# malcolmgreaves/deequ

Measured on AMD Instinct MI355X. Metric: rows/sec (whole node) for fused 16-col profile scan; % of HBM peak BW, higher is better.
Workload: dtype f64+int64+utf8; 1 GPU; C5 fused 16-col profile scan (8 f64 + 4 i64 + 4 utf8, 10% nulls) + state merge + incremental StateLoader append; rows_per_gpu=1000000000, chunk_rows=125000000, analyzers=93, parallelism=row-shard x1

## Files before the change

deequ_amd/csrc/dq_device.h:

```cpp
#pragma once

#include <cstdint>

namespace dq {

constexpr int kBlock = 256;
constexpr int kWaves = kBlock / 64;
constexpr int kRowsPerLane = 8;
constexpr int kRowsPerIter = kBlock * kRowsPerLane;
constexpr int kMaxWG = 4096;
constexpr int kTargetWGs = 8192;
constexpr int kMaxCols = 64;
constexpr int kMaxColTasks = 256;
constexpr int kMaxSchemaCols = 1 << 16;
constexpr int kMaxWhere = 8;
constexpr int kHllCopies = 8;
constexpr int kPredAccCopies = 16;
constexpr int kMaxRoots = 32;
constexpr int kMaxCounters = 32;
constexpr int kMaxInstr = 96;
constexpr int kPredStack = 16;
constexpr int kMaxRegexWords = 32768;

enum ColKind : int32_t {
// ... 77 lines not shown
};

struct alignas(16) ColPartial {
  double n, mean, m2;
  double sum;
  int64_t isum;
  int64_t count;
  int64_t nan_count;
  double fmin, fmax;
  int64_t pinf_count;
  int64_t ninf_count;
  int64_t isum_hi;
};
static_assert(sizeof(ColPartial) == 96, "ColPartial layout");

struct alignas(16) CorrPartial {
  double n, xa, ya, ck, xm, ym, pad0, pad1;
};
static_assert(sizeof(CorrPartial) == 64, "CorrPartial layout");

struct alignas(16) PredPartial {
  int64_t t[kMaxCounters];
  int64_t nn[kMaxCounters];
};

enum PredOp : int32_t {
  PO_ATOM_CMP = 1,
  PO_ATOM_ISNULL = 2,
  PO_ATOM_NOTNULL = 3,
  PO_CONST = 4,
// ... 58 lines not shown
```

deequ_amd/csrc/dq_kernels.hip:

```cpp
#include <hip/hip_runtime.h>

#include <cstdint>
#include <type_traits>

#include "dq_device.h"
#include "dq_hash.h"
#include "dq_decimal.h"
#include "dq_lane.h"
#include "dq_shift.h"

namespace dq {

#define DQ_DEC_TABLE static __constant__ const
#include "dq_dec_tables.inc"
#undef DQ_DEC_TABLE
__device__ __forceinline__ DecTab dec_dev_tab() { return DecTab{kDecP10Lo, kDecP10Hi, kDecRcpHi, kDecRcpLo}; }

typedef uint32_t u32x4 __attribute__((ext_vector_type(4)));

__device__ __forceinline__ uint32_t ld32(const uint8_t* base, int64_t a) {
  return *reinterpret_cast<const uint32_t*>(base + a);
}
__device__ __forceinline__ uint32_t read4(const uint8_t* base, int64_t pos) {
  int64_t a = pos & ~int64_t(3);
// ... 75 lines not shown
__device__ __forceinline__ uint32_t hll_hi_from_fmix(uint64_t b) {
  const uint32_t bl = (uint32_t)b, bh = (uint32_t)(b >> 32);
  return __umulhi(bl, (uint32_t)XP3) + bl * (uint32_t)(XP3 >> 32) + bh * (uint32_t)XP3;
}
__device__ __forceinline__ HllKey hll_key_from_fmix(uint64_t b) {
  const uint32_t hi = hll_hi_from_fmix(b);
  return {(hi >> 21) & 0x7FCu, ffbh_raw(hi << 9)};
}

constexpr int32_t kFloorMin = 13;
__device__ __forceinline__ uint32_t hll_floor_thr(const uint32_t* __restrict__ hll_floor, int32_t slot) {
  if (!hll_floor || slot < 0) return 0u;
  const int32_t qfloor = (int32_t)hll_floor[slot] - 1;
  return qfloor >= kFloorMin ? 1u << (31 - min(qfloor, 22)) : 0u;
}
__device__ __forceinline__ HllKey hll_key_long(uint64_t v) { return hll_key_from_fmix(xxh64_long_head(v)); }
__device__ __forceinline__ HllKey hll_key_int(uint32_t v) { return hll_key_from_fmix(xxh64_int_head(v)); }


struct ColStats {
  double n, mean, m2, sum;
  int64_t isum, count, nan_count;
  double fmin, fmax;
  int64_t pinf, ninf;
  int64_t isum_hi;
};

__device__ __forceinline__ void stats_init(ColStats& s) {
  s.n = 0.0; s.mean = 0.0; s.m2 = 0.0; s.sum = 0.0;
  s.isum = 0; s.count = 0; s.nan_count = 0;
// ... 169 lines not shown
    asm volatile(
        "s_and_saveexec_b64 %[save], %[ma]\n\t"
        "v_add_f64 %[d], %[x], -%[sh]\n\t"
        "v_add_f64 %[sd], %[sd], %[d]\n\t"
        "v_fma_f64 %[sdd], %[d], %[d], %[sdd]\n\t"
        "s_and_b64 exec, %[save], %[mb]\n\t"
        "v_min_f64 %[lo], %[lo], %[x]\n\t"
        "v_max_f64 %[hi], %[hi], %[x]\n\t"
        "s_mov_b64 exec, %[save]"
        : [sd] "+v"(a.sd), [sdd] "+v"(a.sdd), [lo] "+v"(lo), [hi] "+v"(hi), [d] "=&v"(d), [save] "=&s"(save)
        : [x] "v"(x), [sh] "s"(shift), [ma] "s"(ma), [mb] "s"(mb)
        : "scc");
  }
}

template <int KIND, bool STATS, bool HLL, bool FLOOR = false>
__device__ __forceinline__ void numeric_block(const double (&x)[8], const uint64_t (&bits)[8], const uint64_t (&m)[8],
                                              double shift, ColStats& s, LaneMoments& a, int32_t* regs, int32_t& qmin,
                                              uint32_t thr = 0) {
  uint32_t rmin = ~0u;
#pragma unroll
  for (int j = 0; j < 8; ++j) {
    if (STATS) masked_moments<!ck_float(KIND), false>(a, s.fmin, s.fmax, x[j], bits[j], shift, m[j], m[j]);
    if (HLL) {
      if constexpr (FLOOR) {
        const uint64_t b = ck_bytes(KIND) <= 4 ? xxh64_int_head((uint32_t)bits[j]) : xxh64_long_head(bits[j]);
        rmin = min(rmin, hll_hi_from_fmix(b) << 9);
      } else {
        const HllKey key = ck_bytes(KIND) <= 4 ? hll_key_int((uint32_t)bits[j]) : hll_key_long(bits[j]);
        qmin = min(qmin, key.q);
        if (lane_bit(m[j])) atomicMax(reinterpret_cast<int32_t*>(reinterpret_cast<char*>(regs) + key.addr), key.q);
      }
    }
  }
  if (HLL) {
    const bool redo = FLOOR ? rmin < thr : qmin < 0;
    if (__builtin_amdgcn_ballot_w64(redo) != 0) {
#pragma unroll 1
      for (int j = 0; j < 8; ++j) {
        if (lane_bit(m[j])) hll_update(regs, ck_bytes(KIND) <= 4 ? xxh64_int((uint32_t)bits[j]) : xxh64_long(bits[j]));
      }
      qmin = 0;
    }
  }
}

template <int KIND, bool STATS, bool HLL>
__device__ __forceinline__ void float_block_checked(__amdgpu_buffer_rsrc_t vr, const uint32_t* validity,
                                                    const uint32_t* mask, int64_t base, int32_t rem, int32_t vo,
                                                    double shift, ColStats& s, LaneMoments& a, int32_t* regs,
                                                    int64_t& cnt_w, int64_t& nan_v, int64_t& pinf_v, int64_t& ninf_v) {
  constexpr bool kF32 = KIND == CK_F32;
// ... 34 lines not shown
      if (lane_bit(mj)) {
        if (key.q >= 0) atomicMax(reinterpret_cast<int32_t*>(reinterpret_cast<char*>(regs) + key.addr), key.q);
        else hll_update(regs, kF32 ? xxh64_int((uint32_t)b) : xxh64_long(b));
      }
    }
  }
}

template <int K> struct KindT { using T = double; };
template <> struct KindT<CK_I64> { using T = int64_t; };
template <> struct KindT<CK_I32> { using T = int32_t; };
template <> struct KindT<CK_F32> { using T = float; };
template <> struct KindT<CK_I16> { using T = int16_t; };
template <> struct KindT<CK_I8> { using T = int8_t; };

template <int KIND, bool STATS, bool HLL>
__device__ void numeric_range(const void* values, const uint32_t* validity, const uint32_t* mask,
                              int64_t row0, int64_t row1, ColStats& s, int32_t* regs, uint32_t thr = 0) {
  using T = typename KindT<KIND>::T;
  constexpr bool kLazy = ck_float(KIND) && STATS;
  const int lane = threadIdx.x & 63;
  const int wave = __builtin_amdgcn_readfirstlane(threadIdx.x >> 6);
  const T* v = reinterpret_cast<const T*>(values);
  const __amdgpu_buffer_rsrc_t vr = __builtin_amdgcn_make_buffer_rsrc(
      const_cast<T*>(v + row0), (short)0, (int)((row1 - row0) * (int64_t)sizeof(T)), 0x00020000);
  int64_t nan_v = 0, pinf_v = 0, ninf_v = 0;
  int64_t cnt_w = 0;
  LaneMoments a{0.0, 0.0, 0};
  const double shift =
      STATS ? range_shift(validity, mask, row0, row1, lane, [=](int64_t r) { return range_value<KIND>(vr, r - row0); }) : 0.0;
  int32_t qmin = 0;
  const int32_t nr = (int32_t)(row1 - row0);
  auto block_loop = [&](auto floor_form) __attribute__((always_inline)) {
    constexpr bool FLOOR = decltype(floor_form)::value;
    for (int32_t rb = 0; rb < nr; rb += kRowsPerIter) {
      const int64_t base = row0 + rb + wave * 512;
      const int32_t rem = nr - rb - wave * 512;
      const bool full = rb + kRowsPerIter <= nr;
      uint64_t bits[8], m[8];
      double x[8];
      const int32_t vo = (rb + wave * 512 + lane) * (int32_t)sizeof(T);
#pragma unroll
      for (int j = 0; j < 8; ++j) {
        if constexpr (sizeof(T) == 8) {
          const auto w2 = __builtin_amdgcn_raw_buffer_load_b64(vr, vo + j * 512, 0, 2 );
          bits[j] = ((uint64_t)w2[1] << 32) | w2[0];
          if (KIND == CK_F64) x[j] = __builtin_bit_cast(double, bits[j]);
          else x[j] = __builtin_fma((double)(int32_t)w2[1], 4294967296.0, (double)w2[0]);
        } else if constexpr (KIND == CK_F32) {
// ... 9 lines not shown
          x[j] = (double)w;
        }
      }
      block_masks(validity, mask, base, rem, full, m);
      uint64_t nf_any = 0;
      if constexpr (ck_float(KIND) && !kLazy) {
#pragma unroll
        for (int j = 0; j < 8; ++j) nf_any |= __builtin_amdgcn_ballot_w64(!__builtin_isfinite(x[j])) & m[j];
      }
      if (ck_float(KIND) && !kLazy && nf_any != 0) {
        float_block_checked<KIND, STATS, HLL>(vr, validity, mask, base, rem, vo, shift, s, a, regs, cnt_w, nan_v, pinf_v,
                                              ninf_v);
      } else {
#pragma unroll
        for (int j = 0; j < 8; ++j) cnt_w += __builtin_popcountll(m[j]);
        numeric_block<KIND, STATS, HLL, FLOOR>(x, bits, m, shift, s, a, regs, qmin, thr);
      }
    }
  };
  if (HLL && thr != 0) block_loop(std::true_type{});
  else block_loop(std::false_type{});
  if constexpr (kLazy) {
    __shared__ int32_t redo;
    if (threadIdx.x == 0) redo = 0;
    __syncthreads();
    const bool bad = !__builtin_isfinite(a.sd) || !__builtin_isfinite(a.sdd);
    if (__builtin_amdgcn_ballot_w64(bad) != 0 && lane == 0) redo = 1;
    __syncthreads();
    if (redo) {
      if (HLL) {
        for (int i = threadIdx.x; i < 512; i += kBlock) regs[i] = -1;
      }
      stats_init(s);
      a = LaneMoments{0.0, 0.0, 0};
      cnt_w = 0;
      __syncthreads();
// ... 600 lines not shown
  }
  s.count += c;
}

template <int KIND, bool STATS, bool HLL>
__device__ void run_numeric(const ColTask& t, const ScanCols& cols, const ScanBitmaps& bm, int64_t row0, int64_t row1,
                            ColStats& s, int32_t* regs) {
  const uint32_t* mask = t.where >= 0 ? reinterpret_cast<const uint32_t*>(bm.where_bits[t.where]) : nullptr;
  numeric_range<KIND, STATS, HLL>(cols.values[t.col], cols.validity[t.col], mask, row0, row1, s, regs);
}

template <int V, bool LONG>
__device__ __forceinline__ void run_variant(const ColTask& t, const ScanCols& cols, const uint32_t* mask, int64_t row0,
                                            int64_t row1, int64_t n_rows, ColStats& s, int32_t* regs,
                                            const uint64_t* p5, uint32_t* dq, uint32_t* rare, uint32_t* cls,
                                            uint32_t thr) {
  const void* v = cols.values[t.col];
  const uint32_t* val = cols.validity[t.col];
  if constexpr (V == CV_VALIDITY) validity_range(val, mask, row0, row1, s);
  else if constexpr (V == CV_F64_S) numeric_range<CK_F64, true, false>(v, val, mask, row0, row1, s, regs);
  else if constexpr (V == CV_F64_SH) numeric_range<CK_F64, true, true>(v, val, mask, row0, row1, s, regs, thr);
  else if constexpr (V == CV_F64_H) numeric_range<CK_F64, false, true>(v, val, mask, row0, row1, s, regs, thr);
  else if constexpr (V == CV_I64_S) numeric_range<CK_I64, true, false>(v, val, mask, row0, row1, s, regs);
  else if constexpr (V == CV_I64_SH) numeric_range<CK_I64, true, true>(v, val, mask, row0, row1, s, regs, thr);
  else if constexpr (V == CV_I64_H) numeric_range<CK_I64, false, true>(v, val, mask, row0, row1, s, regs, thr);
  else if constexpr (V == CV_I32_S) numeric_range<CK_I32, true, false>(v, val, mask, row0, row1, s, regs);
  else if constexpr (V == CV_I32_SH) numeric_range<CK_I32, true, true>(v, val, mask, row0, row1, s, regs, thr);
  else if constexpr (V == CV_I32_H) numeric_range<CK_I32, false, true>(v, val, mask, row0, row1, s, regs, thr);
  else if constexpr (V == CV_F32_S) numeric_range<CK_F32, true, false>(v, val, mask, row0, row1, s, regs);
  else if constexpr (V == CV_F32_SH) numeric_range<CK_F32, true, true>(v, val, mask, row0, row1, s, regs, thr);
  else if constexpr (V == CV_F32_H) numeric_range<CK_F32, false, true>(v, val, mask, row0, row1, s, regs, thr);
  else if constexpr (V == CV_I16_S) numeric_range<CK_I16, true, false>(v, val, mask, row0, row1, s, regs);
  else if constexpr (V == CV_I16_SH) numeric_range<CK_I16, true, true>(v, val, mask, row0, row1, s, regs, thr);
  else if constexpr (V == CV_I16_H) numeric_range<CK_I16, false, true>(v, val, mask, row0, row1, s, regs, thr);
  else if constexpr (V == CV_I8_S) numeric_range<CK_I8, true, false>(v, val, mask, row0, row1, s, regs);
  else if constexpr (V == CV_I8_SH) numeric_range<CK_I8, true, true>(v, val, mask, row0, row1, s, regs, thr);
  else if constexpr (V == CV_I8_H) numeric_range<CK_I8, false, true>(v, val, mask, row0, row1, s, regs, thr);
  else if constexpr (V == CV_F64_D) float_dtype_range(reinterpret_cast<const double*>(v), val, mask, row0, row1, s);
  else if constexpr (V == CV_F32_D) float_dtype_range(reinterpret_cast<const float*>(v), val, mask, row0, row1, s);
  else if constexpr (V == CV_BOOL) bool_range(reinterpret_cast<const uint32_t*>(v), val, mask, row0, row1, s, regs);
  else if constexpr (V == CV_D128_S) decimal_range<true, false, false>(v, val, mask, row0, row1, s, regs, t.arg);
  else if constexpr (V == CV_D128_SH) decimal_range<true, true, false>(v, val, mask, row0, row1, s, regs, t.arg);
  else if constexpr (V == CV_D128_H) decimal_range<false, true, false>(v, val, mask, row0, row1, s, regs, t.arg);
  else if constexpr (V == CV_D128_D) decimal_range<false, false, true>(v, val, mask, row0, row1, s, regs, t.arg);
  else if constexpr (V == CV_UTF8_H || V == CV_UTF8_D || V == CV_UTF8_HD)
    utf8_range<int32_t, V != CV_UTF8_D, V != CV_UTF8_H, LONG>(
        reinterpret_cast<const uint8_t*>(v), reinterpret_cast<const int32_t*>(cols.offsets[t.col]), val, mask, row0,
        row1, n_rows, s, regs, p5, dq, rare, cls);
  else
    utf8_range<int64_t, V != CV_LUTF8_D, V != CV_LUTF8_H, LONG>(
        reinterpret_cast<const uint8_t*>(v), reinterpret_cast<const int64_t*>(cols.offsets[t.col]), val, mask, row0,
// ... 7 lines not shown
#define DQ_NUM_WAVES 6
#endif
template <int V, bool LONG>
constexpr int kMinWaves = V == CV_UTF8_H && !LONG && DQ_STR_CLS ? 5
                          : V == CV_UTF8_H && DQ_STR_WAVES > 0 ? DQ_STR_WAVES
                          : (V == CV_F64_SH || V == CV_I64_SH) && DQ_NUM_WAVES > 0 ? DQ_NUM_WAVES
                          : V == CV_LUTF8_H && LONG ? 5
                                                    : 1;

template <int V, bool LONG = false>
__global__ __launch_bounds__(kBlock) __attribute__((amdgpu_waves_per_eu(kMinWaves<V, LONG>))) void dq_column_scan(const ColTask* __restrict__ tasks, int32_t ntasks,
                                                         int32_t part_base, ScanCols cols, ScanBitmaps bm,
                                                         int64_t n_rows, int64_t rows_per_range,
                                                         ColPartial* __restrict__ partials,
                                                         uint32_t* __restrict__ hll_acc,
                                                         const uint32_t* __restrict__ hll_floor) {
  constexpr bool kHll = !(V == CV_VALIDITY || V == CV_F64_S || V == CV_I64_S || V == CV_I32_S || V == CV_F64_D ||
                         V == CV_UTF8_D || V == CV_LUTF8_D || V == CV_F32_S || V == CV_I16_S || V == CV_I8_S ||
                         V == CV_F32_D || V == CV_BOOL || V == CV_D128_S || V == CV_D128_D);
  constexpr bool kBool = V == CV_BOOL;
  constexpr bool kStr = V == CV_UTF8_H || V == CV_LUTF8_H || V == CV_UTF8_HD || V == CV_LUTF8_HD;
  __shared__ int32_t regs[kHll ? 512 : 2];
  __shared__ uint64_t p5[kStr ? 256 : 1];
  constexpr uint32_t kDCap = DQ_STR_CLS && (V == CV_UTF8_H || V == CV_LUTF8_H) && !LONG ? kDefCapCls : kDefCap;
  __shared__ uint32_t dfq[kStr ? kWaves * kDefFields * kDCap : 1];
  __shared__ uint32_t rare[kStr ? kWaves : 1];
  constexpr bool kCls = DQ_STR_CLS && (V == CV_UTF8_H || V == CV_LUTF8_H) && !LONG;
  __shared__ __attribute__((aligned(16))) uint32_t clsbuf[kCls ? kWaves * kClsWords : 4];
  __shared__ ColStats red[kWaves];
  const int32_t ti = blockIdx.x % ntasks;
  const int32_t range = blockIdx.x / ntasks;
  const ColTask t = tasks[ti];
  const int64_t row0 = (int64_t)range * rows_per_range;
  int64_t row1 = row0 + rows_per_range;
  if (row1 > n_rows) row1 = n_rows;
  if constexpr (kBool) {
    if (threadIdx.x < 2) regs[threadIdx.x] = 0;
    __syncthreads();
  }
  if constexpr (kHll) {
    for (int i = threadIdx.x; i < 512; i += kBlock) regs[i] = -1;
    if constexpr (kStr) {
      p5[threadIdx.x] = (uint64_t)threadIdx.x * XP5;
      if (threadIdx.x < kWaves) rare[threadIdx.x] = 0;
    }
    __syncthreads();
  }
  ColStats s;
  stats_init(s);
  const uint32_t* mask = t.where >= 0 ? reinterpret_cast<const uint32_t*>(bm.where_bits[t.where]) : nullptr;
  const int32_t wv = kStr ? __builtin_amdgcn_readfirstlane(threadIdx.x >> 6) : 0;
  run_variant<V, LONG>(t, cols, mask, row0, row1, n_rows, s, regs, p5, dfq + wv * kDefFields * kDCap, rare + wv,
                       clsbuf + (kCls ? wv * kClsWords : 0), kHll ? hll_floor_thr(hll_floor, t.hll_slot) : 0u);
  block_reduce_store(s, partials + (size_t)(part_base + ti) * kMaxWG + range, red);
  if constexpr (kStr) {
    if (threadIdx.x == 0 && bm.rare_rows) {
      uint32_t r = 0;
      for (int w = 0; w < kWaves; ++w) r += rare[w];
      if (r) atomicAdd(reinterpret_cast<unsigned long long*>(bm.rare_rows + part_base + ti), (unsigned long long)r);
    }
  }
  if constexpr (kBool) {
    if (threadIdx.x == 0 && t.hll_slot >= 0) {
      uint32_t* dst = hll_acc + ((size_t)t.hll_slot * kHllCopies + (blockIdx.x % kHllCopies)) * 512;
      for (int b = 0; b < 2; ++b) {
        if (!regs[b]) continue;
        const uint64_t x = xxh64_int(b == 0 ? 1u : 0u);
        atomicMax(dst + (uint32_t)(x >> 55), (uint32_t)(hll_q_exact(x) + 1));
      }
// ... 505 lines not shown
      }
    }
    pred_block_out(S, s_ctr, n_counters, s_bmroot, n_bitmaps, bm, wr, inr, n_rows, lane);
  }
  pred_counters_out(pred_lds, wave_words, prog, acc);
}

__global__ __launch_bounds__(kBlock) void dq_finalize(int32_t ncol, int32_t nranges_col,
                                                      const ColPartial* __restrict__ col_part,
                                                      ColPartial* __restrict__ col_acc, int32_t npair, int32_t nranges_pair,
                                                      const CorrPartial* __restrict__ pair_part,
                                                      CorrPartial* __restrict__ pair_acc, int32_t has_pred,
                                                      int32_t nranges_pred, const PredPartial* __restrict__ pred_part,
                                                      PredPartial* __restrict__ pred_acc, FinRanges fr,
                                                      int64_t* __restrict__ rare_dev, int64_t* rare_host,
                                                      int32_t nhll, const uint32_t* __restrict__ hll_acc,
                                                      uint32_t* __restrict__ hll_floor) {
  __shared__ ColStats cs[kBlock];
  __shared__ CorrStats ps[kBlock];
  const int b = blockIdx.x, tid = threadIdx.x;
  if (b < ncol) {
    int32_t nr = nranges_col;
    for (int i = 0; i < fr.n; ++i)
      if (b >= fr.first[i] && b < fr.end[i]) nr = fr.nr[i];
    ColStats s;
    stats_init(s);
    for (int r = tid; r < nr; r += kBlock) stats_merge(s, stats_load(col_part + (size_t)b * kMaxWG + r));
    cs[tid] = s;
    __syncthreads();
    for (int stride = kBlock / 2; stride >= 1; stride >>= 1) {
      if (tid < stride) { ColStats a = cs[tid]; stats_merge(a, cs[tid + stride]); cs[tid] = a; }
      __syncthreads();
// ... 19 lines not shown
    __syncthreads();
    for (int stride = kBlock / 2; stride >= 1; stride >>= 1) {
      if (tid < stride) { CorrStats a = ps[tid]; corr_merge(a, ps[tid + stride]); ps[tid] = a; }
      __syncthreads();
    }
    if (tid == 0) {
      CorrPartial& q = pair_acc[p];
      CorrStats acc = {q.n, q.xa, q.ya, q.ck, q.xm, q.ym};
      corr_merge(acc, ps[0]);
      q.n = acc.n; q.xa = acc.xa; q.ya = acc.ya; q.ck = acc.ck; q.xm = acc.xm; q.ym = acc.ym;
    }
  } else if (b >= ncol + npair + (has_pred ? 1 : 0)) {
    const int slot = b - (ncol + npair + (has_pred ? 1 : 0));
    if (slot >= nhll) return;
    __shared__ uint32_t fmin_w[kWaves];
    const uint32_t* src = hll_acc + (size_t)slot * kHllCopies * 512;
    uint32_t f = ~0u;
    for (int i = tid; i < 512; i += kBlock) {
      uint32_t r = 0;
      for (int c = 0; c < kHllCopies; ++c) r = max(r, src[c * 512 + i]);
      f = min(f, r);
    }
    for (int o = 32; o >= 1; o >>= 1) f = min(f, (uint32_t)__shfl_xor((int)f, o));
    if ((tid & 63) == 0) fmin_w[tid >> 6] = f;
    __syncthreads();
    if (tid == 0) {
      for (int w = 1; w < kWaves; ++w) f = min(f, fmin_w[w]);
      hll_floor[slot] = f;
    }
  } else if (has_pred) {
    static_assert(kBlock % kMaxCounters == 0, "counter layout");
// ... 31 lines not shown
hipError_t launch_pred_scan(const PredProgram* prog, const ScanCols& cols, const ScanBitmaps& bm, int64_t n_rows,
                            int64_t rows_per_range, int32_t nranges, PredPartial* acc, int32_t lds_bytes, hipStream_t st,
                            bool has_regex) {
  if (has_regex)
    hipLaunchKernelGGL(dq_pred_scan<true>, dim3(nranges), dim3(kBlock), (size_t)lds_bytes, st, prog, cols, bm, n_rows,
                       rows_per_range, acc);
  else
    hipLaunchKernelGGL(dq_pred_scan<false>, dim3(nranges), dim3(kBlock), (size_t)lds_bytes, st, prog, cols, bm, n_rows,
                       rows_per_range, acc);
  return hipGetLastError();
}

template <int V>
static void launch_v(const ColTask* tasks, int32_t ntasks, int32_t part_base, const ScanCols& cols,
                     const ScanBitmaps& bm, int64_t n_rows, int64_t rows_per_range, int32_t nranges,
                     ColPartial* partials, uint32_t* hll_acc, const uint32_t* hll_floor, bool long_str,
                     hipStream_t st) {
  constexpr bool kStrHll = V == CV_UTF8_H || V == CV_LUTF8_H || V == CV_UTF8_HD || V == CV_LUTF8_HD;
  if constexpr (kStrHll) {
    if (long_str) {
      hipLaunchKernelGGL((dq_column_scan<V, true>), dim3((uint32_t)ntasks * (uint32_t)nranges), dim3(kBlock), 0, st,
                         tasks, ntasks, part_base, cols, bm, n_rows, rows_per_range, partials, hll_acc, hll_floor);
      return;
    }
  }
  hipLaunchKernelGGL(dq_column_scan<V>, dim3((uint32_t)ntasks * (uint32_t)nranges), dim3(kBlock), 0, st, tasks, ntasks,
                     part_base, cols, bm, n_rows, rows_per_range, partials, hll_acc, hll_floor);
}

hipError_t launch_column_scan(int32_t variant, const ColTask* tasks, int32_t ntasks, int32_t part_base,
                              const ScanCols& cols, const ScanBitmaps& bm, int64_t n_rows, int64_t rows_per_range,
                              int32_t nranges, ColPartial* partials, uint32_t* hll_acc, const uint32_t* hll_floor,
                              bool long_str, hipStream_t st) {
#define DQ_V(V)                                                                                            \
  case V:                                                                                                  \
    launch_v<V>(tasks, ntasks, part_base, cols, bm, n_rows, rows_per_range, nranges, partials, hll_acc, hll_floor, \
                long_str, st);                                                                             \
    break;
  switch (variant) {
    DQ_V(CV_VALIDITY) DQ_V(CV_F64_S) DQ_V(CV_F64_SH) DQ_V(CV_F64_H) DQ_V(CV_I64_S) DQ_V(CV_I64_SH) DQ_V(CV_I64_H)
    DQ_V(CV_I32_S) DQ_V(CV_I32_SH) DQ_V(CV_I32_H) DQ_V(CV_UTF8_H) DQ_V(CV_LUTF8_H)
    DQ_V(CV_UTF8_D) DQ_V(CV_UTF8_HD) DQ_V(CV_LUTF8_D) DQ_V(CV_LUTF8_HD) DQ_V(CV_F64_D)
    DQ_V(CV_F32_S) DQ_V(CV_F32_SH) DQ_V(CV_F32_H) DQ_V(CV_I16_S) DQ_V(CV_I16_SH) DQ_V(CV_I16_H)
    DQ_V(CV_I8_S) DQ_V(CV_I8_SH) DQ_V(CV_I8_H) DQ_V(CV_F32_D) DQ_V(CV_BOOL)
    DQ_V(CV_D128_S) DQ_V(CV_D128_SH) DQ_V(CV_D128_H) DQ_V(CV_D128_D)
    default: return hipErrorInvalidValue;
  }
#undef DQ_V
  return hipGetLastError();
}


hipError_t launch_finalize(int32_t ncol, int32_t nranges_col, const ColPartial* col_part, ColPartial* col_acc,
                           int32_t npair, int32_t nranges_pair, const CorrPartial* pair_part, CorrPartial* pair_acc,
                           int32_t has_pred, int32_t nranges_pred, const PredPartial* pred_part, PredPartial* pred_acc,
                           const FinRanges& fr, int64_t* rare_dev, int64_t* rare_host, int32_t nhll,
                           const uint32_t* hll_acc, uint32_t* hll_floor, hipStream_t st) {
  if (!hll_floor) nhll = 0;
  const uint32_t nb = (uint32_t)(ncol + npair + (has_pred ? 1 : 0) + nhll);
  if (nb == 0) return hipSuccess;
  hipLaunchKernelGGL(dq_finalize, dim3(nb), dim3(kBlock), 0, st, ncol, nranges_col, col_part, col_acc, npair,
                     nranges_pair, pair_part, pair_acc, has_pred, nranges_pred, pred_part, pred_acc, fr, rare_dev,
                     rare_host, nhll, hll_acc, hll_floor);
  return hipGetLastError();
}

hipError_t launch_init_acc(ColPartial* col_acc, int32_t ncol, CorrPartial* pair_acc, int32_t npair, int64_t* rare_dev,
                           hipStream_t st) {
  const int n = ncol > npair ? ncol : npair;
  if (n == 0) return hipSuccess;
  hipLaunchKernelGGL(dq_init_acc, dim3((n + 255) / 256), dim3(256), 0, st, col_acc, ncol, pair_acc, npair, rare_dev);
  return hipGetLastError();
}

}
```

deequ_amd/csrc/dq_plan.cpp:

```cpp
#include <hip/hip_runtime.h>

#include <algorithm>
#include <chrono>
#include <cmath>
#include <cstdarg>
#include <cstdio>
#include <cstdlib>
#include <cstring>
#include <functional>
#include <iterator>
#include <limits>
#include <map>
#include <memory>
#include <string>
#include <tuple>
#include <vector>

#include "dq_device.h"
#include "dq_internal.h"
#include "dq_pred_jit.h"

#ifndef DQ_MIN_RANGE_ROWS
#define DQ_MIN_RANGE_ROWS 16384
#endif
// ... 7 lines not shown
#define DQ_PAIR_ONE_ROUND 1
#endif
#ifndef DQ_PRED_WGS
#define DQ_PRED_WGS 2048
#endif
#include "dq_regex.h"

namespace dq {

hipError_t launch_pred_scan(const PredProgram* prog, const ScanCols& cols, const ScanBitmaps& bm, int64_t n_rows,
                            int64_t rows_per_range, int32_t nranges, PredPartial* acc, int32_t lds_bytes, hipStream_t st,
                            bool has_regex);
hipError_t launch_column_scan(int32_t variant, const ColTask* tasks, int32_t ntasks, int32_t part_base,
                              const ScanCols& cols, const ScanBitmaps& bm, int64_t n_rows, int64_t rows_per_range,
                              int32_t nranges, ColPartial* partials, uint32_t* hll_acc, const uint32_t* hll_floor,
                              bool long_str, hipStream_t st);
hipError_t launch_pair_scan(const PairWG* wgs, int32_t nwg, const ScanCols& cols, const ScanBitmaps& bm,
                            const uint32_t* ones, int64_t n_rows, int64_t rows_per_range, int32_t nranges,
                            CorrPartial* pair_part, ColPartial* col_part, int32_t* redo, bool all_f64, bool ring,
                            bool minmax, hipStream_t st);
hipError_t pair_scan_residency(bool all_f64, bool ring, bool minmax, int32_t* per_cu);
hipError_t launch_finalize(int32_t ncol, int32_t nranges_col, const ColPartial* col_part, ColPartial* col_acc,
                           int32_t npair, int32_t nranges_pair, const CorrPartial* pair_part, CorrPartial* pair_acc,
                           int32_t has_pred, int32_t nranges_pred, const PredPartial* pred_part, PredPartial* pred_acc, const FinRanges& fr, int64_t* rare_dev, int64_t* rare_host,
                           int32_t nhll, const uint32_t* hll_acc, uint32_t* hll_floor, hipStream_t st);
hipError_t launch_init_acc(ColPartial* col_acc, int32_t ncol, CorrPartial* pair_acc, int32_t npair, int64_t* rare_dev,
                           hipStream_t st);

static thread_local char g_err[1024] = "";
static thread_local bool g_capacity = false;

dq_status set_error(dq_status code, const char* fmt, ...) {
  va_list ap;
  va_start(ap, fmt);
  std::vsnprintf(g_err, sizeof(g_err), fmt, ap);
  va_end(ap);
  return code;
}

static dq_status cap_error(const char* fmt, ...) {
// ... 547 lines not shown
  char* h_stage = nullptr;
  int64_t* d_rare_dev = nullptr;
  int64_t* h_rare = nullptr;
  int64_t* d_rare = nullptr;
  std::vector<uint8_t> str_long;
  int32_t str_path = 0;
  int64_t prev_rows = 0;
  size_t h_stage_bytes = 0;
  PredProgram* d_prog = nullptr;
  ColPartial* d_col_part = nullptr;
  CorrPartial* d_pair_part = nullptr;
  PredPartial* d_pred_part = nullptr;
  ColPartial* d_col_acc = nullptr;
  uint32_t* d_hll_acc = nullptr;
  uint32_t* d_hll_floor = nullptr;
  CorrPartial* d_pair_acc = nullptr;
  PredPartial* d_pred_acc = nullptr;
  uint64_t* d_where_bits[kMaxWhere] = {nullptr};
  int64_t where_cap_words = 0;
  uint32_t* d_ones = nullptr;
  int64_t ones_cap_words = 0;

  int64_t total_rows = 0;
  int64_t next_chunk = 0;

  bool timing = false;
  std::vector<hipEvent_t> ev_pool;
  struct Pending { int kernel; hipEvent_t a, b; };
  std::vector<Pending> pending;
  static constexpr int kTimers = 16 + kNumVariants;
// ... 40 lines not shown
  HIP_TRY(fn());
  if (p->timing) {
    HIP_TRY(hipEventRecord(b, st));
    p->pending.push_back({kernel, a, b});
  }
  return DQ_OK;
}

static dq_status free_plan_mem(dq_plan* p) {
  for (auto& q : p->pending) { p->ev_pool.push_back(q.a); p->ev_pool.push_back(q.b); }
  p->pending.clear();
  for (hipEvent_t e : p->ev_pool) (void)hipEventDestroy(e);
  p->ev_pool.clear();
  void* ptrs[] = {p->d_col_tasks, p->d_pair_tasks, p->d_pair_wgs, p->d_prog, p->d_col_part, p->d_pair_part,
                  p->d_pred_part, p->d_col_acc, p->d_hll_acc, p->d_pair_acc, p->d_pred_acc, p->d_regex, p->d_pair_redo,
                  p->d_rare_dev, p->d_hll_floor};
  for (void* q : ptrs)
    if (q) (void)hipFree(q);
  for (int i = 0; i < kMaxWhere; ++i)
    if (p->d_where_bits[i]) (void)hipFree(p->d_where_bits[i]);
  if (p->d_ones) (void)hipFree(p->d_ones);
  if (p->h_rare) (void)hipHostFree(p->h_rare);
  p->h_rare = p->d_rare = nullptr;
  if (p->h_stage) (void)hipHostFree(p->h_stage);
  p->h_stage = nullptr;
  p->h_stage_bytes = 0;
  return DQ_OK;
}

static dq_status reset_acc(dq_plan* p) {
  HIP_TRY(launch_init_acc(p->d_col_acc, (int32_t)p->col_tasks.size(), p->d_pair_acc, (int32_t)p->pair_tasks.size(),
                          p->d_rare_dev, p->stream));
  if (p->n_hll) HIP_TRY(hipMemsetAsync(p->d_hll_acc, 0, (size_t)p->n_hll * kHllCopies * 512 * sizeof(uint32_t), p->stream));
  if (p->n_hll && p->d_hll_floor) HIP_TRY(hipMemsetAsync(p->d_hll_floor, 0, (size_t)p->n_hll * sizeof(uint32_t), p->stream));
  if (p->has_pred) HIP_TRY(hipMemsetAsync(p->d_pred_acc, 0, kPredAccCopies * sizeof(PredPartial), p->stream));
  if (p->total_rows > 0) p->prev_rows = p->total_rows;
  p->total_rows = 0;
  p->next_chunk = 0;
  return DQ_OK;
}

template <typename T>
static dq_status dmalloc(T** ptr, size_t bytes) {
  if (bytes == 0) bytes = 16;
  HIP_TRY(hipMalloc((void**)ptr, bytes));
  return DQ_OK;
}

static void plan_pair_wgs(const dq_plan* p, const PairGroup& g, std::vector<PairWG>& out, std::vector<int>& fused) {
// ... 522 lines not shown
  if (nct && hipHostMalloc(reinterpret_cast<void**>(&p->h_rare), nct * sizeof(int64_t), hipHostMallocMapped) == hipSuccess) {
    std::memset(p->h_rare, 0, nct * sizeof(int64_t));
    void* dp = nullptr;
    if (hipHostGetDevicePointer(&dp, p->h_rare, 0) == hipSuccess) {
      p->d_rare = static_cast<int64_t*>(dp);
    } else {
      (void)hipHostFree(p->h_rare);
      p->h_rare = nullptr;
    }
  }
  (void)hipGetLastError();
  if (dq_status s = dmalloc(&p->d_hll_acc, (size_t)p->n_hll * kHllCopies * 512 * sizeof(uint32_t))) return s;
  const char* floor_env = std::getenv("DQ_HLL_FLOOR");
  if (p->n_hll && !(floor_env && std::strcmp(floor_env, "0") == 0))
    if (dq_status s = dmalloc(&p->d_hll_floor, (size_t)p->n_hll * sizeof(uint32_t))) return s;
  if (dq_status s = dmalloc(&p->d_pair_acc, npt * sizeof(CorrPartial))) return s;
  if (dq_status s = dmalloc(&p->d_pred_acc, kPredAccCopies * sizeof(PredPartial))) return s;
  if (nct) HIP_TRY(hipMemcpyAsync(p->d_col_tasks, p->col_tasks.data(), nct * sizeof(ColTask), hipMemcpyHostToDevice, p->stream));
  if (npt) HIP_TRY(hipMemcpyAsync(p->d_pair_tasks, p->pair_tasks.data(), npt * sizeof(PairTask), hipMemcpyHostToDevice, p->stream));
  if (!p->regex_blob.empty()) {
    if (dq_status s = dmalloc(&p->d_regex, p->regex_blob.size() * sizeof(uint16_t))) return s;
    HIP_TRY(hipMemcpyAsync(p->d_regex, p->regex_blob.data(), p->regex_blob.size() * sizeof(uint16_t),
                           hipMemcpyHostToDevice, p->stream));
  }
  p->prog.regex = p->d_regex;
  p->prog.regex_words = (int32_t)p->regex_blob.size();
  HIP_TRY(hipMemcpyAsync(p->d_prog, &p->prog, sizeof(PredProgram), hipMemcpyHostToDevice, p->stream));
  if (dq_status s = reset_acc(p)) return s;
  HIP_TRY(hipStreamSynchronize(p->stream));
  return DQ_OK;
// ... 522 lines not shown
      return false;
    if (p->str_path != 0) return p->str_path == 2;
    const int64_t rows = p->total_rows > 0 ? p->total_rows : p->prev_rows;
    bool any = false;
    for (int32_t t = g.first; t < g.first + g.count; ++t) {
      if (p->h_rare && rows > 0) p->str_long[t] = __atomic_load_n(p->h_rare + t, __ATOMIC_RELAXED) * 4096 > rows;
      any = any || p->str_long[t];
    }
    return any;
  };
  for (size_t gi = 0; gi < groups.size(); ++gi) {
    const auto& g = groups[gi];
    if (dq_status s = timed(p, 16 + g.variant, p->stream, [&] {
          return launch_column_scan(g.variant, p->d_col_tasks + g.first, g.count, g.first, sc, bm, n_rows,
                                    vr[gi].first, vr[gi].second, p->d_col_part, p->d_hll_acc, p->d_hll_floor,
                                    str_long_of(g), p->stream);
        }))
      return s;
  }
  if (!p->pair_wgs.empty()) {
    const bool ring = pair_ring;
    if (dq_status s = timed(p, 2, p->stream, [&] {
          return launch_pair_scan(p->d_pair_wgs, (int32_t)p->pair_wgs.size(), sc, bm, p->d_ones, n_rows, rpr_pair,
                                  nr_pair, p->d_pair_part, p->d_col_part, p->d_pair_redo, p->pair_all_f64, ring,
                                  p->pair_minmax, p->stream);
        }))
      return s;
  }
  if (dq_status s = timed(p, 3, p->stream, [&] {
        return launch_finalize((int32_t)p->col_tasks.size(), nr_col, p->d_col_part, p->d_col_acc,
                               (int32_t)p->pair_tasks.size(), nr_pair, p->d_pair_part, p->d_pair_acc,
                               0 , nr_pred, p->d_pred_part, p->d_pred_acc,
                               fr, p->d_rare_dev, p->d_rare, p->n_hll, p->d_hll_acc, p->d_hll_floor, p->stream);
      }))
    return s;
  p->total_rows += n_rows;
  return DQ_OK;
}

dq_status dq_finish(dq_plan* p, dq_state* out) {
  if (!p) return set_error(DQ_E_INVALID, "dq_finish: plan is NULL");
  if (!out && !p->specs.empty()) return set_error(DQ_E_INVALID, "dq_finish: out is NULL");
  HIP_TRY(hipSetDevice(p->device));
  if (!p->parts.empty()) {
    std::vector<dq_state> tmp;
    for (size_t k = 0; k < p->parts.size(); ++k) {
      tmp.assign(p->part_specs[k].size(), dq_state{});
      if (dq_status s = dq_finish(p->parts[k], tmp.data())) return s;
// ... 404 lines not shown
```

Measured before the change: 30.12 billion rows/s.

## Replace per-row HLL hashing of narrow-range integer columns with a value-window bitmap

For integer columns that need both stats and HLL, the range of values seen in earlier chunks is used to build a 64K-bit window. Rows whose value falls inside the window set a bit in a shared-memory bitmap instead of being hashed, and the bitmap is merged into global memory. In finalize, the set bits are hashed once into the HLL registers and the window is recentred for the next chunk. This removes per-row xxhash work when the column's integer span is small, at the cost of extra shared memory, atomics, a fallback path for out-of-window rows, and more finalize work.

```diff
diff --git a/deequ_amd/csrc/dq_device.h b/deequ_amd/csrc/dq_device.h
--- a/deequ_amd/csrc/dq_device.h
+++ b/deequ_amd/csrc/dq_device.h
@@ -115,6 +115,17 @@
 };
 static_assert(sizeof(ColPartial) == 96, "ColPartial layout");
 
+constexpr int kHllWinBits = 1 << 16;
+constexpr int kHllWinWords = kHllWinBits / 32;
+struct alignas(16) HllWindow {
+  int64_t lo, hi;
+  int64_t base;
+  uint32_t active;
+  uint32_t seen;
+  uint32_t bits[kHllWinWords];
+};
+static_assert(sizeof(HllWindow) == 32 + 4 * kHllWinWords, "HllWindow layout");
+
 struct alignas(16) CorrPartial {
   double n, xa, ya, ck, xm, ym, pad0, pad1;
 };
diff --git a/deequ_amd/csrc/dq_kernels.hip b/deequ_amd/csrc/dq_kernels.hip
--- a/deequ_amd/csrc/dq_kernels.hip
+++ b/deequ_amd/csrc/dq_kernels.hip
@@ -113,6 +113,10 @@
   const int32_t qfloor = (int32_t)hll_floor[slot] - 1;
   return qfloor >= kFloorMin ? 1u << (31 - min(qfloor, 22)) : 0u;
 }
+struct HllWin {
+  uint32_t* bits = nullptr;
+  uint64_t base = 0;
+};
 __device__ __forceinline__ HllKey hll_key_long(uint64_t v) { return hll_key_from_fmix(xxh64_long_head(v)); }
 __device__ __forceinline__ HllKey hll_key_int(uint32_t v) { return hll_key_from_fmix(xxh64_int_head(v)); }
 
@@ -312,16 +316,22 @@
   }
 }
 
-template <int KIND, bool STATS, bool HLL, bool FLOOR = false>
+template <int KIND, bool STATS, bool HLL, bool FLOOR = false, bool WIN = false>
 __device__ __forceinline__ void numeric_block(const double (&x)[8], const uint64_t (&bits)[8], const uint64_t (&m)[8],
                                               double shift, ColStats& s, LaneMoments& a, int32_t* regs, int32_t& qmin,
-                                              uint32_t thr = 0) {
+                                              uint32_t thr = 0, const HllWin& win = HllWin{}) {
   uint32_t rmin = ~0u;
+  uint64_t outside = 0;
 #pragma unroll
   for (int j = 0; j < 8; ++j) {
     if (STATS) masked_moments<!ck_float(KIND), false>(a, s.fmin, s.fmax, x[j], bits[j], shift, m[j], m[j]);
     if (HLL) {
-      if constexpr (FLOOR) {
+      if constexpr (WIN) {
+        const uint64_t rel = bits[j] - win.base;
+        const uint64_t in = __builtin_amdgcn_ballot_w64(rel < (uint64_t)kHllWinBits);
+        outside |= m[j] & ~in;
+        if (lane_bit(m[j] & in)) atomicOr(win.bits + ((uint32_t)rel >> 5), 1u << ((uint32_t)rel & 31u));
+      } else if constexpr (FLOOR) {
         const uint64_t b = ck_bytes(KIND) <= 4 ? xxh64_int_head((uint32_t)bits[j]) : xxh64_long_head(bits[j]);
         rmin = min(rmin, hll_hi_from_fmix(b) << 9);
       } else {
@@ -333,7 +343,7 @@
   }
   if (HLL) {
     const bool redo = FLOOR ? rmin < thr : qmin < 0;
-    if (__builtin_amdgcn_ballot_w64(redo) != 0) {
+    if (WIN ? outside != 0 : __builtin_amdgcn_ballot_w64(redo) != 0) {
 #pragma unroll 1
       for (int j = 0; j < 8; ++j) {
         if (lane_bit(m[j])) hll_update(regs, ck_bytes(KIND) <= 4 ? xxh64_int((uint32_t)bits[j]) : xxh64_long(bits[j]));
@@ -398,9 +408,10 @@
 template <> struct KindT<CK_I16> { using T = int16_t; };
 template <> struct KindT<CK_I8> { using T = int8_t; };
 
-template <int KIND, bool STATS, bool HLL>
+template <int KIND, bool STATS, bool HLL, bool WIN = false>
 __device__ void numeric_range(const void* values, const uint32_t* validity, const uint32_t* mask,
-                              int64_t row0, int64_t row1, ColStats& s, int32_t* regs, uint32_t thr = 0) {
+                              int64_t row0, int64_t row1, ColStats& s, int32_t* regs, uint32_t thr = 0,
+                              const HllWin& win = HllWin{}) {
   using T = typename KindT<KIND>::T;
   constexpr bool kLazy = ck_float(KIND) && STATS;
   const int lane = threadIdx.x & 63;
@@ -415,8 +426,9 @@
       STATS ? range_shift(validity, mask, row0, row1, lane, [=](int64_t r) { return range_value<KIND>(vr, r - row0); }) : 0.0;
   int32_t qmin = 0;
   const int32_t nr = (int32_t)(row1 - row0);
-  auto block_loop = [&](auto floor_form) __attribute__((always_inline)) {
+  auto block_loop = [&](auto floor_form, auto win_form) __attribute__((always_inline)) {
     constexpr bool FLOOR = decltype(floor_form)::value;
+    constexpr bool WINF = decltype(win_form)::value;
     for (int32_t rb = 0; rb < nr; rb += kRowsPerIter) {
       const int64_t base = row0 + rb + wave * 512;
       const int32_t rem = nr - rb - wave * 512;
@@ -456,12 +468,18 @@
       } else {
 #pragma unroll
         for (int j = 0; j < 8; ++j) cnt_w += __builtin_popcountll(m[j]);
-        numeric_block<KIND, STATS, HLL, FLOOR>(x, bits, m, shift, s, a, regs, qmin, thr);
+        numeric_block<KIND, STATS, HLL, FLOOR, WINF>(x, bits, m, shift, s, a, regs, qmin, thr, win);
       }
     }
   };
-  if (HLL && thr != 0) block_loop(std::true_type{});
-  else block_loop(std::false_type{});
+  if constexpr (WIN) {
+    if (win.bits) block_loop(std::false_type{}, std::true_type{});
+    else if (thr != 0) block_loop(std::true_type{}, std::false_type{});
+    else block_loop(std::false_type{}, std::false_type{});
+  } else {
+    if (HLL && thr != 0) block_loop(std::true_type{}, std::false_type{});
+    else block_loop(std::false_type{}, std::false_type{});
+  }
   if constexpr (kLazy) {
     __shared__ int32_t redo;
     if (threadIdx.x == 0) redo = 0;
@@ -1092,7 +1110,7 @@
 __device__ __forceinline__ void run_variant(const ColTask& t, const ScanCols& cols, const uint32_t* mask, int64_t row0,
                                             int64_t row1, int64_t n_rows, ColStats& s, int32_t* regs,
                                             const uint64_t* p5, uint32_t* dq, uint32_t* rare, uint32_t* cls,
-                                            uint32_t thr) {
+                                            uint32_t thr, const HllWin& win) {
   const void* v = cols.values[t.col];
   const uint32_t* val = cols.validity[t.col];
   if constexpr (V == CV_VALIDITY) validity_range(val, mask, row0, row1, s);
@@ -1100,19 +1118,19 @@
   else if constexpr (V == CV_F64_SH) numeric_range<CK_F64, true, true>(v, val, mask, row0, row1, s, regs, thr);
   else if constexpr (V == CV_F64_H) numeric_range<CK_F64, false, true>(v, val, mask, row0, row1, s, regs, thr);
   else if constexpr (V == CV_I64_S) numeric_range<CK_I64, true, false>(v, val, mask, row0, row1, s, regs);
-  else if constexpr (V == CV_I64_SH) numeric_range<CK_I64, true, true>(v, val, mask, row0, row1, s, regs, thr);
+  else if constexpr (V == CV_I64_SH) numeric_range<CK_I64, true, true, true>(v, val, mask, row0, row1, s, regs, thr, win);
   else if constexpr (V == CV_I64_H) numeric_range<CK_I64, false, true>(v, val, mask, row0, row1, s, regs, thr);
   else if constexpr (V == CV_I32_S) numeric_range<CK_I32, true, false>(v, val, mask, row0, row1, s, regs);
-  else if constexpr (V == CV_I32_SH) numeric_range<CK_I32, true, true>(v, val, mask, row0, row1, s, regs, thr);
+  else if constexpr (V == CV_I32_SH) numeric_range<CK_I32, true, true, true>(v, val, mask, row0, row1, s, regs, thr, win);
   else if constexpr (V == CV_I32_H) numeric_range<CK_I32, false, true>(v, val, mask, row0, row1, s, regs, thr);
   else if constexpr (V == CV_F32_S) numeric_range<CK_F32, true, false>(v, val, mask, row0, row1, s, regs);
   else if constexpr (V == CV_F32_SH) numeric_range<CK_F32, true, true>(v, val, mask, row0, row1, s, regs, thr);
   else if constexpr (V == CV_F32_H) numeric_range<CK_F32, false, true>(v, val, mask, row0, row1, s, regs, thr);
   else if constexpr (V == CV_I16_S) numeric_range<CK_I16, true, false>(v, val, mask, row0, row1, s, regs);
-  else if constexpr (V == CV_I16_SH) numeric_range<CK_I16, true, true>(v, val, mask, row0, row1, s, regs, thr);
+  else if constexpr (V == CV_I16_SH) numeric_range<CK_I16, true, true, true>(v, val, mask, row0, row1, s, regs, thr, win);
   else if constexpr (V == CV_I16_H) numeric_range<CK_I16, false, true>(v, val, mask, row0, row1, s, regs, thr);
   else if constexpr (V == CV_I8_S) numeric_range<CK_I8, true, false>(v, val, mask, row0, row1, s, regs);
-  else if constexpr (V == CV_I8_SH) numeric_range<CK_I8, true, true>(v, val, mask, row0, row1, s, regs, thr);
+  else if constexpr (V == CV_I8_SH) numeric_range<CK_I8, true, true, true>(v, val, mask, row0, row1, s, regs, thr, win);
   else if constexpr (V == CV_I8_H) numeric_range<CK_I8, false, true>(v, val, mask, row0, row1, s, regs, thr);
   else if constexpr (V == CV_F64_D) float_dtype_range(reinterpret_cast<const double*>(v), val, mask, row0, row1, s);
   else if constexpr (V == CV_F32_D) float_dtype_range(reinterpret_cast<const float*>(v), val, mask, row0, row1, s);
@@ -1150,7 +1168,8 @@
                                                          int64_t n_rows, int64_t rows_per_range,
                                                          ColPartial* __restrict__ partials,
                                                          uint32_t* __restrict__ hll_acc,
-                                                         const uint32_t* __restrict__ hll_floor) {
+                                                         const uint32_t* __restrict__ hll_floor,
+                                                         HllWindow* __restrict__ hll_win) {
   constexpr bool kHll = !(V == CV_VALIDITY || V == CV_F64_S || V == CV_I64_S || V == CV_I32_S || V == CV_F64_D ||
                          V == CV_UTF8_D || V == CV_LUTF8_D || V == CV_F32_S || V == CV_I16_S || V == CV_I8_S ||
                          V == CV_F32_D || V == CV_BOOL || V == CV_D128_S || V == CV_D128_D);
@@ -1164,6 +1183,8 @@
   constexpr bool kCls = DQ_STR_CLS && (V == CV_UTF8_H || V == CV_LUTF8_H) && !LONG;
   __shared__ __attribute__((aligned(16))) uint32_t clsbuf[kCls ? kWaves * kClsWords : 4];
   __shared__ ColStats red[kWaves];
+  constexpr bool kWin = V == CV_I64_SH || V == CV_I32_SH || V == CV_I16_SH || V == CV_I8_SH;
+  __shared__ uint32_t wbits[kWin ? kHllWinWords : 1];
   const int32_t ti = blockIdx.x % ntasks;
   const int32_t range = blockIdx.x / ntasks;
   const ColTask t = tasks[ti];
@@ -1182,13 +1203,31 @@
     }
     __syncthreads();
   }
+  HllWin win;
+  if constexpr (kWin) {
+    if (hll_win && t.hll_slot >= 0 && hll_win[t.hll_slot].active) {
+      win.bits = wbits;
+      win.base = (uint64_t)hll_win[t.hll_slot].base;
+      for (int i = threadIdx.x; i < kHllWinWords; i += kBlock) wbits[i] = 0;
+      __syncthreads();
+    }
+  }
   ColStats s;
   stats_init(s);
   const uint32_t* mask = t.where >= 0 ? reinterpret_cast<const uint32_t*>(bm.where_bits[t.where]) : nullptr;
   const int32_t wv = kStr ? __builtin_amdgcn_readfirstlane(threadIdx.x >> 6) : 0;
   run_variant<V, LONG>(t, cols, mask, row0, row1, n_rows, s, regs, p5, dfq + wv * kDefFields * kDCap, rare + wv,
-                       clsbuf + (kCls ? wv * kClsWords : 0), kHll ? hll_floor_thr(hll_floor, t.hll_slot) : 0u);
+                       clsbuf + (kCls ? wv * kClsWords : 0), kHll ? hll_floor_thr(hll_floor, t.hll_slot) : 0u, win);
   block_reduce_store(s, partials + (size_t)(part_base + ti) * kMaxWG + range, red);
+  if constexpr (kWin) {
+    if (win.bits) {
+      uint32_t* dst = hll_win[t.hll_slot].bits;
+      for (int i = threadIdx.x; i < kHllWinWords; i += kBlock) {
+        const uint32_t w = wbits[i];
+        if (w != 0 && (w & ~__builtin_nontemporal_load(dst + i)) != 0) atomicOr(dst + i, w);
+      }
+    }
+  }
   if constexpr (kStr) {
     if (threadIdx.x == 0 && bm.rare_rows) {
       uint32_t r = 0;
@@ -1724,8 +1763,10 @@
                                                       int32_t nranges_pred, const PredPartial* __restrict__ pred_part,
                                                       PredPartial* __restrict__ pred_acc, FinRanges fr,
                                                       int64_t* __restrict__ rare_dev, int64_t* rare_host,
-                                                      int32_t nhll, const uint32_t* __restrict__ hll_acc,
-                                                      uint32_t* __restrict__ hll_floor) {
+                                                      int32_t nhll, uint32_t* __restrict__ hll_acc,
+                                                      uint32_t* __restrict__ hll_floor,
+                                                      HllWindow* __restrict__ hll_win,
+                                                      const int32_t* __restrict__ hll_win_task) {
   __shared__ ColStats cs[kBlock];
   __shared__ CorrStats ps[kBlock];
   const int b = blockIdx.x, tid = threadIdx.x;
@@ -1775,7 +1816,77 @@
     const int slot = b - (ncol + npair + (has_pred ? 1 : 0));
     if (slot >= nhll) return;
     __shared__ uint32_t fmin_w[kWaves];
-    const uint32_t* src = hll_acc + (size_t)slot * kHllCopies * 512;
+    uint32_t* src = hll_acc + (size_t)slot * kHllCopies * 512;
+    const int32_t wt = hll_win && hll_win_task ? hll_win_task[slot] : -1;
+    __shared__ uint32_t wreg[512];
+    __shared__ double wlo[kWaves], whi[kWaves];
+    if (wt >= 0) {
+      HllWindow& w = hll_win[slot];
+      const int32_t task = wt & 0xFFFFFF;
+      const bool is64 = (wt >> 24) & 1;
+      for (int i = tid; i < 512; i += kBlock) wreg[i] = 0;
+      __syncthreads();
+      const uint64_t base = (uint64_t)w.base;
+      for (int i = tid; i < kHllWinWords; i += kBlock) {
+        uint32_t word = w.bits[i];
+        if (word == 0) continue;
+        w.bits[i] = 0;
+        while (word) {
+          const int bit = __builtin_ctz(word);
+          word &= word - 1;
+          const uint64_t v = base + (uint64_t)(i * 32 + bit);
+          const uint64_t x = is64 ? xxh64_long(v) : xxh64_int((uint32_t)v);
+          atomicMax(&wreg[(uint32_t)(x >> 55)], (uint32_t)(hll_q_exact(x) + 1));
+        }
+      }
+      int32_t nr = nranges_col;
+      for (int i = 0; i < fr.n; ++i)
+        if (task >= fr.first[i] && task < fr.end[i]) nr = fr.nr[i];
+      double clo = __longlong_as_double(0x7FF0000000000000ll), chi = -clo;
+      for (int r = tid; r < nr; r += kBlock) {
+        const ColPartial& q = col_part[(size_t)task * kMaxWG + r];
+        clo = hw_min(clo, q.fmin);
+        chi = hw_max(chi, q.fmax);
+      }
+      for (int o = 32; o >= 1; o >>= 1) {
+        clo = hw_min(clo, __shfl_xor(clo, o));
+        chi = hw_max(chi, __shfl_xor(chi, o));
+      }
+      if ((tid & 63) == 0) { wlo[tid >> 6] = clo; whi[tid >> 6] = chi; }
+      __syncthreads();
+      for (int i = tid; i < 512; i += kBlock)
+        if (wreg[i] > src[i]) src[i] = wreg[i];
+      if (tid == 0) {
+        for (int k = 1; k < kWaves; ++k) { clo = hw_min(clo, wlo[k]); chi = hw_max(chi, whi[k]); }
+        int64_t lo = w.lo, hi = w.hi;
+        uint32_t seen = w.seen;
+        if (clo <= chi) {
+          const auto sat = [](double d) -> int64_t {
+            return d >= 9223372036854775808.0 ? INT64_MAX : d <= -9223372036854775808.0 ? INT64_MIN : (int64_t)d;
+          };
+          const int64_t l = sat(clo), h = sat(chi);
+          lo = seen && lo < l ? lo : l;
+          hi = seen && hi > h ? hi : h;
+          seen = 1;
+          w.lo = lo;
+          w.hi = hi;
+          w.seen = 1;
+        }
+        const uint64_t span = (uint64_t)hi - (uint64_t)lo;
+        const bool act = seen && span < (uint64_t)kHllWinBits;
+        if (act) {
+          const int64_t half = (int64_t)(((uint64_t)kHllWinBits - 1 - span) / 2);
+          int64_t bs = lo < INT64_MIN + half ? INT64_MIN : lo - half;
+          bs &= ~(int64_t)31;
+          if ((uint64_t)hi - (uint64_t)bs > (uint64_t)kHllWinBits - 1) bs = hi - (kHllWinBits - 1);
+          if (bs > INT64_MAX - (kHllWinBits - 1)) bs = INT64_MAX - (kHllWinBits - 1);
+          w.base = bs;
+        }
+        w.active = act ? 1u : 0u;
+      }
+      __syncthreads();
+    }
+    if (!hll_floor) return;
     uint32_t f = ~0u;
     for (int i = tid; i < 512; i += kBlock) {
       uint32_t r = 0;
@@ -1837,28 +1948,29 @@
 template <int V>
 static void launch_v(const ColTask* tasks, int32_t ntasks, int32_t part_base, const ScanCols& cols,
                      const ScanBitmaps& bm, int64_t n_rows, int64_t rows_per_range, int32_t nranges,
-                     ColPartial* partials, uint32_t* hll_acc, const uint32_t* hll_floor, bool long_str,
-                     hipStream_t st) {
+                     ColPartial* partials, uint32_t* hll_acc, const uint32_t* hll_floor, HllWindow* hll_win,
+                     bool long_str, hipStream_t st) {
   constexpr bool kStrHll = V == CV_UTF8_H || V == CV_LUTF8_H || V == CV_UTF8_HD || V == CV_LUTF8_HD;
   if constexpr (kStrHll) {
     if (long_str) {
       hipLaunchKernelGGL((dq_column_scan<V, true>), dim3((uint32_t)ntasks * (uint32_t)nranges), dim3(kBlock), 0, st,
-                         tasks, ntasks, part_base, cols, bm, n_rows, rows_per_range, partials, hll_acc, hll_floor);
+                         tasks, ntasks, part_base, cols, bm, n_rows, rows_per_range, partials, hll_acc, hll_floor,
+                         hll_win);
       return;
     }
   }
   hipLaunchKernelGGL(dq_column_scan<V>, dim3((uint32_t)ntasks * (uint32_t)nranges), dim3(kBlock), 0, st, tasks, ntasks,
-                     part_base, cols, bm, n_rows, rows_per_range, partials, hll_acc, hll_floor);
+                     part_base, cols, bm, n_rows, rows_per_range, partials, hll_acc, hll_floor, hll_win);
 }
 
 hipError_t launch_column_scan(int32_t variant, const ColTask* tasks, int32_t ntasks, int32_t part_base,
                               const ScanCols& cols, const ScanBitmaps& bm, int64_t n_rows, int64_t rows_per_range,
                               int32_t nranges, ColPartial* partials, uint32_t* hll_acc, const uint32_t* hll_floor,
-                              bool long_str, hipStream_t st) {
+                              HllWindow* hll_win, bool long_str, hipStream_t st) {
 #define DQ_V(V)                                                                                            \
   case V:                                                                                                  \
     launch_v<V>(tasks, ntasks, part_base, cols, bm, n_rows, rows_per_range, nranges, partials, hll_acc, hll_floor, \
-                long_str, st);                                                                             \
+                hll_win, long_str, st);                                                                    \
     break;
   switch (variant) {
     DQ_V(CV_VALIDITY) DQ_V(CV_F64_S) DQ_V(CV_F64_SH) DQ_V(CV_F64_H) DQ_V(CV_I64_S) DQ_V(CV_I64_SH) DQ_V(CV_I64_H)
@@ -1878,13 +1990,14 @@
                            int32_t npair, int32_t nranges_pair, const CorrPartial* pair_part, CorrPartial* pair_acc,
                            int32_t has_pred, int32_t nranges_pred, const PredPartial* pred_part, PredPartial* pred_acc,
                            const FinRanges& fr, int64_t* rare_dev, int64_t* rare_host, int32_t nhll,
-                           const uint32_t* hll_acc, uint32_t* hll_floor, hipStream_t st) {
-  if (!hll_floor) nhll = 0;
+                           uint32_t* hll_acc, uint32_t* hll_floor, HllWindow* hll_win, const int32_t* hll_win_task,
+                           hipStream_t st) {
+  if (!hll_floor && !hll_win) nhll = 0;
   const uint32_t nb = (uint32_t)(ncol + npair + (has_pred ? 1 : 0) + nhll);
   if (nb == 0) return hipSuccess;
   hipLaunchKernelGGL(dq_finalize, dim3(nb), dim3(kBlock), 0, st, ncol, nranges_col, col_part, col_acc, npair,
                      nranges_pair, pair_part, pair_acc, has_pred, nranges_pred, pred_part, pred_acc, fr, rare_dev,
-                     rare_host, nhll, hll_acc, hll_floor);
+                     rare_host, nhll, hll_acc, hll_floor, hll_win, hll_win_task);
   return hipGetLastError();
 }
 
diff --git a/deequ_amd/csrc/dq_plan.cpp b/deequ_amd/csrc/dq_plan.cpp
--- a/deequ_amd/csrc/dq_plan.cpp
+++ b/deequ_amd/csrc/dq_plan.cpp
@@ -45,7 +45,7 @@
 hipError_t launch_column_scan(int32_t variant, const ColTask* tasks, int32_t ntasks, int32_t part_base,
                               const ScanCols& cols, const ScanBitmaps& bm, int64_t n_rows, int64_t rows_per_range,
                               int32_t nranges, ColPartial* partials, uint32_t* hll_acc, const uint32_t* hll_floor,
-                              bool long_str, hipStream_t st);
+                              HllWindow* hll_win, bool long_str, hipStream_t st);
 hipError_t launch_pair_scan(const PairWG* wgs, int32_t nwg, const ScanCols& cols, const ScanBitmaps& bm,
                             const uint32_t* ones, int64_t n_rows, int64_t rows_per_range, int32_t nranges,
                             CorrPartial* pair_part, ColPartial* col_part, int32_t* redo, bool all_f64, bool ring,
@@ -54,7 +54,8 @@
 hipError_t launch_finalize(int32_t ncol, int32_t nranges_col, const ColPartial* col_part, ColPartial* col_acc,
                            int32_t npair, int32_t nranges_pair, const CorrPartial* pair_part, CorrPartial* pair_acc,
                            int32_t has_pred, int32_t nranges_pred, const PredPartial* pred_part, PredPartial* pred_acc, const FinRanges& fr, int64_t* rare_dev, int64_t* rare_host,
-                           int32_t nhll, const uint32_t* hll_acc, uint32_t* hll_floor, hipStream_t st);
+                           int32_t nhll, uint32_t* hll_acc, uint32_t* hll_floor, HllWindow* hll_win,
+                           const int32_t* hll_win_task, hipStream_t st);
 hipError_t launch_init_acc(ColPartial* col_acc, int32_t ncol, CorrPartial* pair_acc, int32_t npair, int64_t* rare_dev,
                            hipStream_t st);
 
@@ -632,6 +633,8 @@
   ColPartial* d_col_acc = nullptr;
   uint32_t* d_hll_acc = nullptr;
   uint32_t* d_hll_floor = nullptr;
+  HllWindow* d_hll_win = nullptr;
+  int32_t* d_hll_win_task = nullptr;
   CorrPartial* d_pair_acc = nullptr;
   PredPartial* d_pred_acc = nullptr;
   uint64_t* d_where_bits[kMaxWhere] = {nullptr};
@@ -702,7 +705,7 @@
   p->ev_pool.clear();
   void* ptrs[] = {p->d_col_tasks, p->d_pair_tasks, p->d_pair_wgs, p->d_prog, p->d_col_part, p->d_pair_part,
                   p->d_pred_part, p->d_col_acc, p->d_hll_acc, p->d_pair_acc, p->d_pred_acc, p->d_regex, p->d_pair_redo,
-                  p->d_rare_dev, p->d_hll_floor};
+                  p->d_rare_dev, p->d_hll_floor, p->d_hll_win, p->d_hll_win_task};
   for (void* q : ptrs)
     if (q) (void)hipFree(q);
   for (int i = 0; i < kMaxWhere; ++i)
@@ -721,6 +724,7 @@
                           p->d_rare_dev, p->stream));
   if (p->n_hll) HIP_TRY(hipMemsetAsync(p->d_hll_acc, 0, (size_t)p->n_hll * kHllCopies * 512 * sizeof(uint32_t), p->stream));
   if (p->n_hll && p->d_hll_floor) HIP_TRY(hipMemsetAsync(p->d_hll_floor, 0, (size_t)p->n_hll * sizeof(uint32_t), p->stream));
+  if (p->n_hll && p->d_hll_win) HIP_TRY(hipMemsetAsync(p->d_hll_win, 0, (size_t)p->n_hll * sizeof(HllWindow), p->stream));
   if (p->has_pred) HIP_TRY(hipMemsetAsync(p->d_pred_acc, 0, kPredAccCopies * sizeof(PredPartial), p->stream));
   if (p->total_rows > 0) p->prev_rows = p->total_rows;
   p->total_rows = 0;
@@ -1273,6 +1277,22 @@
   const char* floor_env = std::getenv("DQ_HLL_FLOOR");
   if (p->n_hll && !(floor_env && std::strcmp(floor_env, "0") == 0))
     if (dq_status s = dmalloc(&p->d_hll_floor, (size_t)p->n_hll * sizeof(uint32_t))) return s;
+  const char* win_env = std::getenv("DQ_HLL_WINDOW");
+  if (p->n_hll && !(win_env && std::strcmp(win_env, "0") == 0)) {
+    std::vector<int32_t> win_task((size_t)p->n_hll, -1);
+    bool any = false;
+    for (size_t t = 0; t < nct; ++t) {
+      const ColTask& ct = p->col_tasks[t];
+      if (ct.variant != CV_I64_SH && ct.variant != CV_I32_SH && ct.variant != CV_I16_SH && ct.variant != CV_I8_SH) continue;
+      win_task[ct.hll_slot] = (int32_t)t | (ct.variant == CV_I64_SH ? 1 << 24 : 0);
+      any = true;
+    }
+    if (any) {
+      if (dq_status s = dmalloc(&p->d_hll_win, (size_t)p->n_hll * sizeof(HllWindow))) return s;
+      if (dq_status s = dmalloc(&p->d_hll_win_task, (size_t)p->n_hll * sizeof(int32_t))) return s;
+      HIP_TRY(hipMemcpy(p->d_hll_win_task, win_task.data(), win_task.size() * sizeof(int32_t), hipMemcpyHostToDevice));
+    }
+  }
   if (dq_status s = dmalloc(&p->d_pair_acc, npt * sizeof(CorrPartial))) return s;
   if (dq_status s = dmalloc(&p->d_pred_acc, kPredAccCopies * sizeof(PredPartial))) return s;
   if (nct) HIP_TRY(hipMemcpyAsync(p->d_col_tasks, p->col_tasks.data(), nct * sizeof(ColTask), hipMemcpyHostToDevice, p->stream));
@@ -1825,7 +1845,7 @@
     if (dq_status s = timed(p, 16 + g.variant, p->stream, [&] {
           return launch_column_scan(g.variant, p->d_col_tasks + g.first, g.count, g.first, sc, bm, n_rows,
                                     vr[gi].first, vr[gi].second, p->d_col_part, p->d_hll_acc, p->d_hll_floor,
-                                    str_long_of(g), p->stream);
+                                    p->d_hll_win, str_long_of(g), p->stream);
         }))
       return s;
   }
@@ -1842,7 +1862,8 @@
         return launch_finalize((int32_t)p->col_tasks.size(), nr_col, p->d_col_part, p->d_col_acc,
                                (int32_t)p->pair_tasks.size(), nr_pair, p->d_pair_part, p->d_pair_acc,
                                0 , nr_pred, p->d_pred_part, p->d_pred_acc,
-                               fr, p->d_rare_dev, p->d_rare, p->n_hll, p->d_hll_acc, p->d_hll_floor, p->stream);
+                               fr, p->d_rare_dev, p->d_rare, p->n_hll, p->d_hll_acc, p->d_hll_floor, p->d_hll_win,
+                               p->d_hll_win_task, p->stream);
       }))
     return s;
   p->total_rows += n_rows;
```

Measured after the change: 30.41 billion rows/s, median of 6. About the same (+1.0%).
